# panosporf99/real-time-mobility-heatmap

Measured on AMD Instinct MI355X. Metric: events/sec H3-snapped+window-aggregated (res 8) at 1/2/4/8 GPUs; % HBM peak, higher is better.
Workload: dtype f64

## Files before the change

real-time-mobility-heatmap_amd/csrc/api_batch.h:

```cpp
#pragma once

int32_t hm_abi_version(void) { return HM_ABI_VERSION; }

int hm_create(const hm_config *cfg, hm_ctx **out) {
    g_create_err.clear();
    if (!cfg || !out) { g_create_err = "null argument"; return HM_E_INVALID; }
    if (cfg->abi_version != HM_ABI_VERSION) { g_create_err = "ABI version mismatch"; return HM_E_INVALID; }
    if (cfg->h3_res < 0 || cfg->h3_res > 15) { g_create_err = "h3_res out of range"; return HM_E_INVALID; }
    if (cfg->tile_us < 1000000 || cfg->watermark_delay_ms < 0) { g_create_err = "bad tile/watermark"; return HM_E_INVALID; }
    if (cfg->shard_count < 0 || cfg->shard_count > 64 || cfg->shard_rank < 0 ||
        (cfg->shard_count > 0 && cfg->shard_rank >= cfg->shard_count) || (cfg->shard_count == 0 && cfg->shard_rank != 0)) {
        g_create_err = "bad shard_rank/shard_count";
        return HM_E_INVALID;
    }
    int ndev = 0;
    if (hipGetDeviceCount(&ndev) != hipSuccess || ndev <= 0) {
        (void)hipGetLastError();
        g_create_err = "no HIP device available (the mobheat hot path requires an MI355X GPU)";
        return HM_E_HIP;
    }
    if (cfg->device < 0 || cfg->device >= ndev) { g_create_err = "device ordinal out of range"; return HM_E_INVALID; }
    hm_ctx *ctx = new hm_ctx();
    ctx->cfg = *cfg;
    ctx->device = cfg->device;
// ... 17 lines not shown
        if (hipEventCreate(&e) != hipSuccess) { ctx->err = "event"; return fail("create"); }
    if (hipEventCreateWithFlags(&ctx->winfo_ev, hipEventDisableTiming) != hipSuccess) { ctx->err = "event"; return fail("create"); }
    for (auto &e : ctx->h2d_ev)
        if (hipEventCreateWithFlags(&e, hipEventDisableTiming) != hipSuccess) { ctx->err = "event"; return fail("create"); }
    for (auto &e : ctx->export_ev)
        if (hipEventCreateWithFlags(&e, hipEventDisableTiming) != hipSuccess) { ctx->err = "event"; return fail("create"); }
    for (auto &e : ctx->stm_ev)
        if (hipEventCreateWithFlags(&e, hipEventDisableTiming) != hipSuccess) { ctx->err = "event"; return fail("create"); }
    if (hipFuncSetAttribute((const void *)k_merge_owned<EventRec, false>, hipFuncAttributeMaxDynamicSharedMemorySize, MO_TAG_MAX) != hipSuccess ||
        hipFuncSetAttribute((const void *)k_merge_owned<EventRec, true>, hipFuncAttributeMaxDynamicSharedMemorySize, MO_TAG_MAX) != hipSuccess ||
        hipFuncSetAttribute((const void *)k_merge_owned<EventRec, true, true>, hipFuncAttributeMaxDynamicSharedMemorySize, MO_TAG_MAX) != hipSuccess ||
        hipFuncSetAttribute((const void *)k_merge_owned<SortedRec, true, true>, hipFuncAttributeMaxDynamicSharedMemorySize, MO_TAG_MAX) != hipSuccess ||
        hipFuncSetAttribute((const void *)k_merge_owned<SortedRec, false>, hipFuncAttributeMaxDynamicSharedMemorySize, MO_TAG_MAX) != hipSuccess ||
        hipFuncSetAttribute((const void *)k_merge_owned<SortedRec, true>, hipFuncAttributeMaxDynamicSharedMemorySize, MO_TAG_MAX) != hipSuccess ||
        hipFuncSetAttribute((const void *)k_merge_owned<EventRec, false, false, true>, hipFuncAttributeMaxDynamicSharedMemorySize, MO_TAG_MAX) != hipSuccess ||
        hipFuncSetAttribute((const void *)k_merge_owned<EventRec, true, false, true>, hipFuncAttributeMaxDynamicSharedMemorySize, MO_TAG_MAX) != hipSuccess ||
        hipFuncSetAttribute((const void *)k_merge_owned<EventRec, true, true, true>, hipFuncAttributeMaxDynamicSharedMemorySize, MO_TAG_MAX) != hipSuccess) {
        ctx->err = "merge LDS attribute";
        return fail("create");
    }
    for (auto &e : ctx->ev)
        if (hipEventCreate(&e) != hipSuccess) { ctx->err = "event"; return fail("create"); }
    if (upload_tables() != hipSuccess) { ctx->err = "tables"; return fail("create"); }
    for (int variant = 0; variant < 2; variant++) {
        const void *kern = variant ? (const void *)k_ingest<true> : (const void *)k_ingest<false>;
        int per_cu = 0, cus = 0;
        if (hipOccupancyMaxActiveBlocksPerMultiprocessor(&per_cu, kern, IG_THREADS, 0) != hipSuccess ||
            hipDeviceGetAttribute(&cus, hipDeviceAttributeMultiprocessorCount, ctx->device) != hipSuccess) {
            ctx->err = "occupancy query";
            return fail("create");
        }
        hipFuncAttributes fa{};
        if (hipFuncGetAttributes(&fa, kern) == hipSuccess && fa.sharedSizeBytes > 0)
            per_cu = std::min<int>(per_cu, (int)(163840 / fa.sharedSizeBytes));
        if (variant) per_cu = std::min(per_cu, 2);
        if (const char *m = getenv("MOBHEAT_INGEST_WG_PER_CU")) {
            int w = 0, cap = 0;
            (void)hipOccupancyMaxActiveBlocksPerMultiprocessor(&cap, kern, IG_THREADS, 0);
            if (fa.sharedSizeBytes > 0) cap = std::min<int>(cap, (int)(163840 / fa.sharedSizeBytes));
            w = atoi(m);
            if (w > 0) per_cu = std::max(1, std::min(cap, w));
        }
        if (getenv("MOBHEAT_DEBUG"))
            fprintf(stderr, "mobheat: k_ingest<%d> %d blocks/CU x %d CUs (LDS %zu B, %d VGPRs)\n", variant, per_cu, cus,
                    fa.sharedSizeBytes, fa.numRegs);
        (variant ? ctx->ingest_grid_bin : ctx->ingest_grid) = std::max(1, per_cu) * std::max(1, cus);
        ctx->n_cus = std::max(1, cus);
    }
    if (const char *m = getenv("MOBHEAT_INGEST_MODE"))
        ctx->ingest_mode = !strcmp(m, "direct") ? 1 : !strcmp(m, "table") ? 2 : !strcmp(m, "binned") ? 3 : 0;
    if (const char *m = getenv("MOBHEAT_MERGE_GRID")) ctx->merge_grid = std::max(0, atoi(m));
    if (const char *m = getenv("MOBHEAT_DEDUP_STREAM")) ctx->dedup_main = !strcmp(m, "main");
    if (const char *m = getenv("MOBHEAT_DEDUP_EARLY")) ctx->early_ok = strcmp(m, "0") != 0;
    if (const char *m = getenv("MOBHEAT_OFFSETS_EARLY")) ctx->offsets_early = strcmp(m, "0") != 0;
    if (const char *m = getenv("MOBHEAT_STAGE_SELF")) ctx->self_hold_ok = strcmp(m, "copy") != 0;
    if (const char *m = getenv("MOBHEAT_DEDUP_DENSE")) ctx->dense_ok = strcmp(m, "0") != 0;
    if (const char *m = getenv("MOBHEAT_COOP_PREDICT")) ctx->coop_predict = strcmp(m, "0") != 0;
    if (const char *m = getenv("MOBHEAT_SUBBINS")) ctx->subbins_mode = !strcmp(m, "0") ? 0 : !strcmp(m, "1") ? 1 : 2;
    if (const char *m = getenv("MOBHEAT_PIPELINE")) ctx->pipe_mode = !strcmp(m, "auto") ? -1 : std::max(0, std::min(atoi(m), hm_ctx::PIPE_MAX));
    if (const char *m = getenv("MOBHEAT_TEST_SLAB_CAP")) ctx->test_slab_cap = (unsigned)std::max(0, atoi(m));
    if (hipMalloc(&ctx->d_wreg, REG_BLOCK_BYTES) != hipSuccess || !(ctx->d_wcount = ctx->d_wreg + WREG_SLOTS + 1) ||
        !(ctx->d_st = (DevStats *)(ctx->d_wreg + 2 * (WREG_SLOTS + 1))) ||
        hipHostMalloc(&ctx->h_wreg, REG_BLOCK_BYTES, hipHostMallocDefault) != hipSuccess ||
        !(ctx->h_wcount = ctx->h_wreg + WREG_SLOTS + 1) || !(ctx->h_st = (DevStats *)(ctx->h_wreg + 2 * (WREG_SLOTS + 1))) ||
        hipMalloc(&ctx->d_winfo, (WREG_SLOTS + 1) * sizeof(WInfo) + sizeof(WiCacheImg)) != hipSuccess ||
        hipHostMalloc(&ctx->h_winfo, (WREG_SLOTS + 1) * sizeof(WInfo) + sizeof(WiCacheImg), hipHostMallocDefault) != hipSuccess ||
        hipMemset(ctx->d_winfo, 0, (WREG_SLOTS + 1) * sizeof(WInfo)) != hipSuccess ||
        hipMemset(ctx->d_winfo + WREG_SLOTS + 1, 0xff, sizeof(WiCacheImg)) != hipSuccess) {
        ctx->err = "window registry alloc";
        return fail("create");
// ... 125 lines not shown
    if (ctx->stream) (void)hipStreamDestroy(ctx->stream);
    delete ctx;
}

const char *hm_last_error(const hm_ctx *ctx) { return ctx ? ctx->err.c_str() : g_create_err.c_str(); }

int hm_last_timings(const hm_ctx *ctx, double *ms, int32_t n) {
    if (!ctx || !ms) return HM_E_INVALID;
    for (int i = 0; i < n && i < 8; i++) ms[i] = ctx->timings[i];
    for (int i = 8; i < n && i < 14; i++) ms[i] = ctx->host_ms[i - 8];
    return HM_OK;
}

int64_t hm_state_version(const hm_ctx *ctx) { return ctx ? (int64_t)ctx->seq : -1; }

int hm_last_counts(const hm_ctx *ctx, int64_t *c, int32_t n) {
    if (!ctx || !c) return HM_E_INVALID;
    for (int i = 0; i < n && i < 6; i++) c[i] = ctx->last_counts[i];
    if (n > 6) c[6] = ctx->n_allocs;
    if (n > 7) c[7] = ctx->n_frees;
    if (n > 8) c[8] = ctx->last_binned;
    if (n > 9) c[9] = ctx->staged ? ctx->stage_self_recs : 0;
    if (n > 10) c[10] = ctx->staged ? 0 : ctx->last_pipe_chunks;
    return HM_OK;
}


int hm_process_batch(hm_ctx *ctx, int64_t epoch_id, const hm_batch_in *in, int32_t out_memory, hm_batch_out *out) {
    if (!ctx || !in || !out || in->n < 0) return ctx ? set_err(ctx, HM_E_INVALID, "bad argument") : HM_E_INVALID;
    if (in->n > MAX_BATCH_ROWS) return set_err(ctx, HM_E_INVALID, "batch of %lld events exceeds %lld", (long long)in->n, (long long)MAX_BATCH_ROWS);
    if (in->n > 0 && (!in->lat || !in->lon || !in->ts_us || !in->vkey))
        return set_err(ctx, HM_E_INVALID, "lat, lon, ts_us and vkey are required");
    if (ctx->shard_count > 1)
        return set_err(ctx, HM_E_STATE, "a context of shard %d of %d runs the stage API (its state is that shard's keys)",
                       ctx->shard_rank, ctx->shard_count);
    HIPCHK(ctx, hipSetDevice(ctx->device));
    host_batch_begin(ctx);
    const BatchClock clock_(ctx);
    memset(out, 0, sizeof(*out));
    ctx->gmap_ready = false;
    ctx->epoch = epoch_id;
    ctx->last_n_latest = -1;
    ctx->staged = false;
    ctx->stage = 0;
    int rc;
    int64_t late_wm = ctx->cfg.late_uses_prev_watermark ? ctx->wm_prev : ctx->wm_cur;
    Inputs I;
    I.n = in->n;
    if ((rc = stage_inputs(ctx, in, &I.lat, &I.lon, &I.ts, &I.sp, &I.sv, &I.vk, &I.rv))) return rc;
    const bool sub = ctx->subbins_mode == 1 || (ctx->subbins_mode == 2 && ctx->merge_coop);
    const bool early = ctx->early_ok && !ctx->dedup_main;
    const int K = pipe_chunks_for(ctx, I);
    bool piped = false;
    ctx->last_pipe_chunks = 0;
    if (K > 1) {
        bool to_table = false;
        if ((rc = process_pipelined(ctx, I, late_wm, sub, K, early, to_table))) return rc;
        piped = !to_table;
    } else if ((rc = phase_local(ctx, I, late_wm, true, sub, early, ctx->offsets_early))) {
        return rc;
    }
    DevStats s1 = *ctx->h_st;
    const int64_t n_agg = (int64_t)s1.n_valid - (int64_t)s1.n_late;
    const bool table = !piped && choose_table(ctx, n_agg, s1.sample_max_run);
    ctx->last_table = table;
    ctx->dedup_side = s1.dedup_retry == 0 && !ctx->dedup_main;
    if (ctx->dedup_early && !ctx->dedup_side)
        HIPCHK(ctx, hipStreamWaitEvent(ctx->stream, ctx->side_ev[2], 0));
    if (ctx->dedup_side && !ctx->dedup_early) {
        HIPCHK(ctx, hipEventRecord(ctx->side_ev[0], ctx->stream));
        HIPCHK(ctx, hipStreamWaitEvent(ctx->side_stream, ctx->side_ev[0], 0));
        if ((rc = launch_side_dedup(ctx, &I))) return rc;
    }
    if (table) {
        int64_t n_parts = 0;
        if ((rc = phase_table(ctx, I, n_agg, &n_parts))) return rc;
        HIPCHK(ctx, hipEventRecord(ctx->ev[2], ctx->stream));
        if ((rc = merge_partials(ctx, (const TilePartial *)ctx->partials.p, n_parts))) return rc;
    } else if (!piped) {
        HIPCHK(ctx, hipEventRecord(ctx->ev[2], ctx->stream));
        if ((rc = merge_events(ctx, I, n_agg))) return rc;
    }
    if (!ctx->dedup_side) {
        if ((rc = phase_dedup(ctx, &I, nullptr, I.n, true))) return rc;
    } else {
// ... 38 lines not shown
```

real-time-mobility-heatmap_amd/csrc/host_batch.h:

```cpp
#pragma once

constexpr int64_t BIN_MIN_ROWS = int64_t(1) << 22;
static bool prev_says_table(const hm_ctx *ctx) {
    return ctx->prev_keys > 0 && ctx->prev_keys <= (int64_t)AG_BINS * (AG_SLOTS / 2) && ctx->prev_agg_rows >= 8 * ctx->prev_keys;
}
static bool choose_binned(const hm_ctx *ctx, int64_t n) {
    if (ctx->ingest_mode) return ctx->ingest_mode == 3;
    return n >= BIN_MIN_ROWS && !prev_says_table(ctx);
}
static unsigned slab_cap_for(int64_t n, double skew, int64_t nbins) {
    const int64_t m = (n + nbins - 1) / nbins;
    const int64_t c = std::min<int64_t>(std::max<int64_t>(m + m / 4 + 256, (int64_t)(skew * 1.1 * (double)m) + 256), n + 256);
    return (unsigned)std::min<int64_t>((c + 1) & ~int64_t(1), (int64_t)UINT32_MAX / 2);
}

static int launch_side_dedup(hm_ctx *ctx, const Inputs *I);
static int bin_offsets(hm_ctx *ctx);
static int prepare_local(hm_ctx *ctx, int64_t n, int64_t late_wm_ms, bool bin, bool sub) {
    int rc;
    if (ctx->dedup_early) HIPCHK(ctx, hipStreamWaitEvent(ctx->stream, ctx->side_ev[2], 0));
    ctx->dedup_early = false;
    if ((rc = ensure(ctx, ctx->flags, n)) || (rc = ensure(ctx, ctx->win, n)) || (rc = ensure(ctx, ctx->rows, n * 8)) ||
        (rc = ensure(ctx, ctx->keys, n * 8)) || (rc = ensure(ctx, ctx->slow, n * sizeof(unsigned int))))
        return rc;
// ... 12 lines not shown
        }
    }
    ctx->keys_partial = bin;
    ctx->keys_late_us = late_wm_ms * 1000;
    ctx->sub_bits = bin && sub ? SUB_BITS : 0;
    const int nbins = RP_BINS << ctx->sub_bits;
    ctx->slab_cap = bin ? slab_cap_for(n, ctx->bin_skew, nbins) : 0;
    if (bin && ctx->test_slab_cap) ctx->slab_cap = std::min(ctx->slab_cap, ctx->test_slab_cap);
    ctx->binned = false;
    ctx->bin_offsets_ready = false;
    if ((rc = ensure(ctx, ctx->bin_cur, ((RP_BINS << SUB_BITS) + 1) * 4))) return rc;
    if (bin && (rc = ensure(ctx, ctx->parts_sorted, ((size_t)nbins * ctx->slab_cap + 64) * sizeof(EventRec)))) return rc;
    {
        const int nw = 2 * (WREG_SLOTS + 1);
        hipLaunchKernelGGL(k_batch_reset, dim3((std::max(nw, nbins + 1) + 255) / 256), dim3(256), 0, ctx->stream,
                           (unsigned long long *)ctx->d_st, ctx->d_scratch + SLOW_WORD, ctx->d_scratch + GIVEUP_WORD, ctx->d_wreg,
                           nw, (unsigned *)ctx->bin_cur.p, nbins + 1);
        HIPCHK(ctx, hipGetLastError());
    }
    return HM_OK;
}

static void launch_ingest(hm_ctx *ctx, const Inputs &I, int64_t a, int64_t b, bool bin, int64_t late_wm_ms) {
    const int blocks = (int)std::min<int64_t>((b - a + IG_THREADS - 1) / IG_THREADS, bin ? ctx->ingest_grid_bin : ctx->ingest_grid);
    auto kern = bin ? k_ingest<true> : k_ingest<false>;
    hipLaunchKernelGGL(kern, dim3(std::max(blocks, 1)), dim3(IG_THREADS), 0, ctx->stream, I.lat, I.lon, I.ts, I.rv, I.vk, a, b,
                       ctx->cfg.h3_res, make_floor_div(ctx->cfg.tile_us), late_wm_ms * 1000, (uint8_t *)ctx->flags.p,
                       (uint64_t *)ctx->keys.p, ctx->dfused.tab, ctx->dfused.cap - 1, (unsigned int *)ctx->dfused.used.p,
                       ctx->d_scratch + ctx->dfused.used_word, (unsigned int *)ctx->slow.p, ctx->d_scratch + SLOW_WORD,
                       ctx->d_scratch + GIVEUP_WORD, ctx->d_wreg, ctx->d_wcount, ctx->d_st, I.sp, I.sv,
                       (unsigned *)ctx->bin_cur.p, bin ? (EventRec *)ctx->parts_sorted.p : nullptr, ctx->slab_cap,
                       (unsigned long long *)ctx->dense.p, ctx->dense_cap, ctx->sub_bits, hs_stride(I.n) - 1);
}

static int phase_local(hm_ctx *ctx, const Inputs &I, int64_t late_wm_ms, bool allow_bin = false, bool sub = false,
                       bool early_dedup = false, bool offsets = false) {
    int64_t n = I.n;
    int rc;
    const bool bin = allow_bin && n > 0 && choose_binned(ctx, n);
    if ((rc = prepare_local(ctx, n, late_wm_ms, bin, sub))) return rc;
    const int nbins = RP_BINS << ctx->sub_bits;
    HIPCHK(ctx, hipEventRecord(ctx->ev[0], ctx->stream));
    if (n > 0) {
        const int nch = ctx->n_h2d ? (int)std::min<int64_t>(hm_ctx::H2D_CHUNKS, std::max<int64_t>(1, n >> 22)) : 1;
        if (ctx->n_h2d) {
            HIPCHK(ctx, hipEventRecord(ctx->h2d_ev[0], ctx->stream));
            HIPCHK(ctx, hipStreamWaitEvent(ctx->copy_stream, ctx->h2d_ev[0], 0));
        }
        for (int c = 0; c < nch; c++) {
            const int64_t a = n * c / nch, b = n * (c + 1) / nch;
            if (ctx->n_h2d) {
                for (int q = 0; q < ctx->n_h2d; q++) {
                    const hm_ctx::H2D &h = ctx->h2d[q];
                    HIPCHK(ctx, hipMemcpyAsync((uint8_t *)h.dst + a * h.el, (const uint8_t *)h.src + a * h.el, (b - a) * h.el,
                                               hipMemcpyHostToDevice, ctx->copy_stream));
// ... 31 lines not shown
        unsigned long long tot = 0, mx = 0;
        for (int b = 0; b < nbins; b++) { tot += ctx->h_bincur[b]; mx = std::max<unsigned long long>(mx, ctx->h_bincur[b]); }
        if (tot) ctx->bin_skew = std::max(1.0, (double)mx * nbins / (double)tot);
    }
    if (ctx->h_st->win_overflow)
        return set_err(ctx, HM_E_OVERFLOW, "more than %d distinct windows in one micro-batch (%llu rows)", WREG_SLOTS,
                       ctx->h_st->win_overflow);
    ctx->binned = bin && ctx->h_st->bin_overflow == 0;
    if (ctx->h_st->vkey_max1) ctx->vkey_bound = (int64_t)ctx->h_st->vkey_max1;
    return HM_OK;
}

static int keys_complete(hm_ctx *ctx, const Inputs &I) {
    if (!ctx->keys_partial) return HM_OK;
    ctx->keys_partial = false;
    if (I.n == 0) return HM_OK;
    const int blocks = (int)std::min<int64_t>((I.n + IG_THREADS - 1) / IG_THREADS, ctx->ingest_grid);
    hipLaunchKernelGGL((k_ingest<false, true>), dim3(blocks), dim3(IG_THREADS), 0, ctx->stream, I.lat, I.lon, I.ts, I.rv, I.vk,
                       (int64_t)0, I.n, ctx->cfg.h3_res, make_floor_div(ctx->cfg.tile_us), ctx->keys_late_us,
                       (uint8_t *)ctx->flags.p, (uint64_t *)ctx->keys.p, ctx->dfused.tab, ctx->dfused.cap - 1,
                       (unsigned int *)ctx->dfused.used.p, ctx->d_scratch + ctx->dfused.used_word, (unsigned int *)ctx->slow.p,
                       ctx->d_scratch + SLOW_WORD, ctx->d_scratch + GIVEUP_WORD, ctx->d_wreg, ctx->d_wcount, ctx->d_st, I.sp,
                       I.sv, (unsigned *)ctx->bin_cur.p, (EventRec *)nullptr, 0u, (unsigned long long *)ctx->dense.p, 0ull, 0u,
                       (int64_t)0);
    HIPCHK(ctx, hipGetLastError());
    return HM_OK;
}

static bool choose_table(const hm_ctx *ctx, int64_t n_agg, unsigned long long sample_max_run) {
    if (ctx->ingest_mode) return ctx->ingest_mode == 2;
    if (n_agg < (int64_t(1) << 16)) return false;
    if (sample_max_run >= (unsigned long long)(HS_SAMPLE / 256)) return true;
    return prev_says_table(ctx);
}

static int phase_table(hm_ctx *ctx, const Inputs &I, int64_t n_agg, int64_t *n_parts) {
    int rc;
    const int64_t n = I.n;
    if ((rc = keys_complete(ctx, I))) return rc;
    if ((rc = ensure(ctx, ctx->partials, std::max<int64_t>(n_agg, 1) * sizeof(TilePartial)))) return rc;
    const int nsub = AG_BINS * AG_SUB;
    if (ctx->agg_cap == 0)
        ctx->agg_cap = (unsigned)std::min<int64_t>(std::max<int64_t>(4096, n_agg / (2 * nsub)), int64_t(1) << 30);
    if ((rc = ensure(ctx, ctx->agg_bucket, (size_t)nsub * ctx->agg_cap * sizeof(AggRec))) ||
        (rc = ensure(ctx, ctx->agg_cursor, (size_t)nsub * 8)))
        return rc;
    HIPCHK(ctx, hipMemsetAsync(ctx->agg_cursor.p, 0, (size_t)nsub * 8, ctx->stream));
// ... 278 lines not shown
```

real-time-mobility-heatmap_amd/csrc/host_ctx.h:

```cpp
#pragma once

struct DevBuf {
    void *p = nullptr;
    size_t bytes = 0;
};

struct Inputs {
    const double *lat, *lon, *sp;
    const int64_t *ts;
    const uint8_t *sv, *rv;
    const uint64_t *vk;
    int64_t n;
};

struct hm_ctx {
    hm_config cfg;
    int device = 0;
    hipStream_t stream = nullptr;
    std::string err;
    hipEvent_t ev[11] = {};
    static constexpr int H2D_CHUNKS = 16;
    hipStream_t copy_stream = nullptr;
    hipStream_t side_stream = nullptr;
    hipEvent_t side_ev[4] = {};
// ... 33 lines not shown
    unsigned long long export_dump_seq = 0;
    static constexpr int STM_PIECES = 64;
    hipEvent_t stm_ev[STM_PIECES] = {};
    int stm_pieces = 0;
    int64_t stm_piece = 0, stm_total = 0;
    static constexpr int EXPORT_SLICES = 64;
    hipEvent_t export_ev[EXPORT_SLICES] = {};
    DevBuf parts_regrow_sorted;
    DevBuf stage_meta, stage_C, stage_P, stage_SO, stage_SP, stage_T, cands_recv, stage_tmp;
    DevBuf gapbuf;
    unsigned long long seq = 0;
    struct DedupTable {
        DedupSlot *tab = nullptr;
        unsigned long long cap = 0;
        DevBuf used;
        bool dirty = false;
        int used_word = 0;
    } dfused, dfull;
    DedupTable *dlast = nullptr;
    int64_t dedup_seen = 0;
    int64_t n_partials_merged = 0;
    int ingest_grid = 0;
    int ingest_grid_bin = 0;
    int64_t last_binned = 0;
    int n_cus = 0;
    int ingest_mode = 0;
    int merge_grid = 0;
    int64_t prev_agg_rows = 0, prev_keys = 0;
    bool merge_coop = false;
    bool coop_predict = true;
    bool last_table = false;
    int64_t last_counts[6] = {0, 0, 0, 0, 0, 0};
    int64_t n_allocs = 0, n_frees = 0;
    int64_t table_evicted = 0;
    struct Dict {
        DevBuf tab, slot_of, occ, slots, code_of_slot, clen, coff, cbytes, btot, boff;
        int64_t last_codes = 0;
        int64_t n_codes = 0;
        void *h_off = nullptr, *h_bytes = nullptr;
        size_t h_off_cap = 0, h_bytes_cap = 0;
    };
    DevBuf jd_bytes, jd_offs, jd_scratch, jd_lat, jd_lon, jd_ts, jd_speed, jd_sv, jd_rv, jd_vkey, jd_poff, jd_plen, jd_voff,
        jd_vlen, jd_un, jd_unrows, jd_patch;
    std::vector<int64_t> jd_unsup;
    int64_t jd_n = -1, jd_np = 0, jd_nv = 0;
    Dict jd_prov, jd_veh;
// ... 808 lines not shown
```

real-time-mobility-heatmap_amd/csrc/host_pipe.h:

```cpp
#pragma once

constexpr int PIPE_CHUNKS = 4;
constexpr int64_t PIPE_MIN_ROWS = int64_t(1) << 24;

static int pipe_chunks_for(const hm_ctx *ctx, const Inputs &I) {
    if (ctx->pipe_mode == 0 || I.n <= 0) return 0;
    if (!choose_binned(ctx, I.n)) return 0;
    if (ctx->pipe_mode > 0) return ctx->pipe_mode >= 2 && I.n >= ctx->pipe_mode ? ctx->pipe_mode : 0;
    return I.n >= PIPE_MIN_ROWS ? PIPE_CHUNKS : 0;
}

static bool g_pipe_debug = getenv("MOBHEAT_PIPE_DEBUG") && getenv("MOBHEAT_PIPE_DEBUG")[0] == '1';
#define PIPE_STEP(ctx, what, k)                                                                                   \
    do {                                                                                                          \
        if (g_pipe_debug) {                                                                                       \
            const hipError_t e_ = hipDeviceSynchronize();                                                         \
            const hipError_t l_ = hipGetLastError();                                                              \
            fprintf(stderr, "[mobheat pipe] %s chunk %d: %s\n", what, (int)(k), hipGetErrorString(e_ ? e_ : l_)); \
            if (e_ || l_) return set_err(ctx, HM_E_HIP, "pipelined batch: %s of chunk %d: %s", what, (int)(k),  \
                                         hipGetErrorString(e_ ? e_ : l_));                                        \
        }                                                                                                         \
    } while (0)

static hipError_t ev_sync(hm_ctx *ctx, hipEvent_t e, int site) {
// ... 37 lines not shown
    return HM_OK;
}

static void pipe_batch_stats(hm_ctx *ctx, int nbins) {
    unsigned long long tot = 0, mx = 0;
    for (int b = 0; b < nbins; b++) { tot += ctx->h_bincur[b]; mx = std::max<unsigned long long>(mx, ctx->h_bincur[b]); }
    if (tot) ctx->bin_skew = std::max(1.0, (double)mx * nbins / (double)tot);
    if (ctx->h_st->vkey_max1) ctx->vkey_bound = (int64_t)ctx->h_st->vkey_max1;
}

static int pipe_overflow_rest(hm_ctx *ctx, const Inputs &I, int K, int k) {
    int rc;
    const int64_t n = I.n, a = n * k / K;
    unsigned long long *plO = (unsigned long long *)ctx->pl_O.p;
    unsigned *plN = (unsigned *)ctx->pl_cnt.p;
    HIPCHK(ctx, hipStreamSynchronize(ctx->merge_stream));
    const int blocks = (int)std::min<int64_t>((n - a + IG_THREADS - 1) / IG_THREADS, ctx->ingest_grid);
    hipLaunchKernelGGL((k_ingest<false, true>), dim3(std::max(blocks, 1)), dim3(IG_THREADS), 0, ctx->stream, I.lat, I.lon, I.ts,
                       I.rv, I.vk, a, n, ctx->cfg.h3_res, make_floor_div(ctx->cfg.tile_us), ctx->keys_late_us,
                       (uint8_t *)ctx->flags.p, (uint64_t *)ctx->keys.p, ctx->dfused.tab, ctx->dfused.cap - 1,
                       (unsigned int *)ctx->dfused.used.p, ctx->d_scratch + ctx->dfused.used_word, (unsigned int *)ctx->slow.p,
                       ctx->d_scratch + SLOW_WORD, ctx->d_scratch + GIVEUP_WORD, ctx->d_wreg, ctx->d_wcount, ctx->d_st, I.sp,
                       I.sv, (unsigned *)ctx->bin_cur.p, (EventRec *)nullptr, 0u, (unsigned long long *)ctx->dense.p, 0ull, 0u,
                       (int64_t)0);
    HIPCHK(ctx, hipGetLastError());
    PIPE_STEP(ctx, "overflow: keys", k);
    ctx->keys_partial = false;
    if (k == 0) {
        int r;
        if ((r = merge_begin(ctx, n, true))) return r;
        HIPCHK(ctx, hipEventRecord(ctx->ev[3], ctx->stream));
    } else if ((rc = gens_sync_counts(ctx))) {
        return rc;
    }
    std::vector<WinCount> census;
    census_of_registry(ctx, census);
    ctx->batch_windows.clear();
    if ((rc = gens_prepare(ctx, census, true)) || (rc = winfo_upload(ctx, true))) return rc;
    Inputs Ik = I;
    Ik.lat += a; Ik.lon += a; Ik.ts += a; Ik.vk += a;
    if (Ik.sp) Ik.sp += a;
    if (Ik.sv) Ik.sv += a;
    if (Ik.rv) Ik.rv += a;
    Ik.n = n - a;
    int64_t ntiles = 1;
    PIPE_STEP(ctx, "overflow: tables", k);
    if ((rc = ev_partition(ctx, (const uint64_t *)ctx->keys.p + a, n - a, &Ik, ntiles))) return rc;
// ... 203 lines not shown
```

real-time-mobility-heatmap_amd/csrc/k_ingest.h:

```cpp
#pragma once

#define HM_SNAP_ATTR __attribute__((amdgpu_waves_per_eu(6)))
__global__ __launch_bounds__(256) void k_cells(const double *__restrict__ lat, const double *__restrict__ lon, int64_t n,
                                               int res, uint64_t *__restrict__ out, unsigned int *__restrict__ slow,
                                               unsigned long long *n_slow) {
    const int64_t stride = (int64_t)gridDim.x * blockDim.x;
    for (int64_t base = (int64_t)blockIdx.x * blockDim.x; base < n; base += stride) {
        const int64_t i = base + threadIdx.x;
        bool exc = false;
        if (i < n) {
            uint64_t c;
            exc = !latLngToCellFast(lat[i], lon[i], res, c_tab, c);
            out[i] = c;
        }
        const unsigned long long pos = wave_append(exc, n_slow);
        if (exc) slow[pos] = (unsigned int)i;
    }
}
__global__ __launch_bounds__(256) void k_cells_exact(const double *__restrict__ lat, const double *__restrict__ lon,
                                                     int res, uint64_t *__restrict__ out, const unsigned int *__restrict__ slow,
                                                     const unsigned long long *n_slow) {
    const int64_t m = (int64_t)*n_slow;
    for (int64_t q = (int64_t)blockIdx.x * blockDim.x + threadIdx.x; q < m; q += (int64_t)gridDim.x * blockDim.x) {
        const unsigned i = slow[q];
        out[i] = latLngToCellDeg(lat[i], lon[i], res, c_tab);
    }
}

constexpr unsigned long long DEDUP_FUSED_PROBES = 32;
constexpr int IG_THREADS = 256;

__device__ __forceinline__ void wave_count_slots(bool pred, int slot, unsigned *cnt) {
    unsigned long long pend = __ballot(pred);
    while (pend) {
        const int leader = __ffsll((long long)pend) - 1;
        const int s = __shfl(slot, leader, 64);
        const unsigned long long m = __ballot(pred && slot == s);
        if (lane_id() == leader) atomicAdd(&cnt[s], (unsigned)__popcll(m));
        pend &= ~m;
    }
}

constexpr int HS_SAMPLE = 4096, HS_THREADS = 1024, HS_SLOTS = 2 * HS_SAMPLE;
__host__ __device__ inline int64_t hs_stride(int64_t n) {
    int64_t s = 1;
    while (s * 2 <= n / HS_SAMPLE) s *= 2;
    return s;
}
template <bool kBin, bool kKeys = false>
__global__ __launch_bounds__(IG_THREADS) HM_SNAP_ATTR void k_ingest(
    const double *__restrict__ lat, const double *__restrict__ lon, const int64_t *__restrict__ ts,
    const uint8_t *__restrict__ row_valid, const uint64_t *__restrict__ vkey, int64_t i_begin, int64_t n, int res_arg, FloorDiv wdiv,
    int64_t late_end_us, uint8_t *__restrict__ flags_out, uint64_t *__restrict__ keys_out, DedupSlot *dtab,
    unsigned long long dmask, unsigned int *dused, unsigned long long *n_dused, unsigned int *__restrict__ slow,
    unsigned long long *n_slow, unsigned long long *dgiveup, unsigned long long *wreg, unsigned long long *wcount,
    DevStats *st, const double *__restrict__ speed, const uint8_t *__restrict__ speed_valid, unsigned *__restrict__ bin_cur,
    EventRec *__restrict__ slabs, unsigned slab_cap, unsigned long long *__restrict__ dense, unsigned long long dense_cap,
    unsigned sub_bits, int64_t smask) {
    static_assert(!(kBin && kKeys), "k_ingest: kKeys runs unbinned");
    const int res = res_arg;
    __shared__ WinCacheL WC;
    __shared__ double Fc[20][3], Fu[20][2][3];
    __shared__ unsigned dskip;
    __shared__ long long tmax_l[IG_THREADS];
    __shared__ long long vmax_l[IG_THREADS];
    for (int k = threadIdx.x; k < 60; k += IG_THREADS) (&Fc[0][0])[k] = (&c_tab.faceCenterPoint[0][0])[k];
    for (int k = threadIdx.x; k < 120; k += IG_THREADS) (&Fu[0][0][0])[k] = (&c_tab.fastU[res & 1][0][0][0])[k];
    __shared__ H3BaseTables BT;
    for (int k = threadIdx.x; k < 20 * 27; k += IG_THREADS) BT.fijkPacked[k] = c_tab.fijkPacked[k];
    for (int k = threadIdx.x; k < 122; k += IG_THREADS) BT.bcdPacked[k] = c_tab.bcdPacked[k];
    for (int k = threadIdx.x; k < AP7_QUAD; k += IG_THREADS) BT.ap7Quad[k] = c_tab.ap7Quad[k];
    for (int k = threadIdx.x; k < AP7_PAIR; k += IG_THREADS) BT.ap7Pair[k] = c_tab.ap7Pair[k];
    wc_init(WC);
    if (threadIdx.x == 0) dskip = 0;
    __syncthreads();
    const int64_t tile_us = wdiv.d;
    unsigned nvalid = 0, nlate = 0, bad = 0, wover = 0, binover = 0;
    tmax_l[threadIdx.x] = INT64_MIN;
    vmax_l[threadIdx.x] = 0;
    bool dretry = false;
    int round = 0;
    const int64_t gstride = (int64_t)gridDim.x * IG_THREADS;
    double nla = 0.0, nlo = 0.0;
    int64_t nt = 0;
    unsigned long long nv = EMPTY_VKEY;
    uint8_t nrv = 1;
    {
        const int64_t i0 = i_begin + (int64_t)blockIdx.x * IG_THREADS + threadIdx.x;
        if (i0 < n) {
            nla = __builtin_nontemporal_load(&lat[i0]);
            nlo = __builtin_nontemporal_load(&lon[i0]);
            nv = __builtin_nontemporal_load(&vkey[i0]);
            if (row_valid) nrv = __builtin_nontemporal_load(&row_valid[i0]);
        }
    }
    for (int64_t base = i_begin + (int64_t)blockIdx.x * IG_THREADS; base < n; base += gstride, round++) {
        const int64_t i = base + threadIdx.x;
        const bool in = i < n;
        const double la = nla, lo = nlo;
        const int64_t t = in ? __builtin_nontemporal_load(&ts[i]) : 0;
        (void)nt;
        uint64_t spb = 0;
        uint8_t svb = 0;
        if constexpr (kBin) {
            typedef __attribute__((address_space(1))) const uint64_t gcu64;
            typedef __attribute__((address_space(1))) const uint8_t gcu8;
            const int64_t j = in ? i : n - 1;
            spb = __builtin_nontemporal_load((gcu64 *)(speed ? (const uint64_t *)&speed[j] : (const uint64_t *)&g_zero_double));
            svb = __builtin_nontemporal_load((gcu8 *)(speed_valid ? &speed_valid[j] : speed ? &g_one_byte : &g_zero_byte));
        }
        const unsigned long long v = nv;
        const bool rv = nrv != 0;
        {
            const int64_t j = i + gstride < n ? i + gstride : n - 1;
            nla = __builtin_nontemporal_load(&lat[j]);
            nlo = __builtin_nontemporal_load(&lon[j]);
            nv = __builtin_nontemporal_load(&vkey[j]);
            nrv = __builtin_nontemporal_load(
                (__attribute__((address_space(1))) const uint8_t *)(row_valid ? &row_valid[j] : &g_one_byte));
// ... 42 lines not shown
        if (dd && dv) {
            const long long cur = (long long)(dn ^ DENSE_SIGN);
            cand = t >= cur;
            if (t > cur) atomicMax(&dense[v], (unsigned long long)t ^ DENSE_SIGN);
        } else if (dd) {
            long long cur = d0.maxts;
            if (d0.vkey == v) dh = (long long)dh0;
            else dh = find_or_claim_vkey_ts(dtab, dmask, v, claimed, DEDUP_FUSED_PROBES, cur);
            if (dh < 0) {
                if (!dretry) atomicExch(dgiveup, 1ull);
                dretry = true;
            } else {
                cand = t >= cur || claimed;
                if (t > cur) atomicMax(&dtab[dh].maxts, (long long)t);
            }
        }
        const bool agg = (fl & F_AGG) != 0;
        const uint64_t key = agg ? ekey_make(exc ? 0 : cell, (unsigned)widx) : 0;
        if (in) {
            if constexpr (!kKeys) flags_out[i] = fl | (cand ? F_CAND : 0);
            if (kKeys ? !exc : !kBin || exc || (i & smask) == 0) keys_out[i] = key;
        }
        if constexpr (kBin) {
            if (agg && !exc) {
                uint64_t inner = wslot >= 0 ? __hip_atomic_load(&WC.inner[wslot], __ATOMIC_RELAXED, __HIP_MEMORY_SCOPE_WORKGROUP) : 0;
                if (inner == 0) {
                    inner = window_inner(ws);
                    if (wslot >= 0) __hip_atomic_store(&WC.inner[wslot], inner, __ATOMIC_RELAXED, __HIP_MEMORY_SCOPE_WORKGROUP);
                }
                const uint64_t h = mix64(cell ^ inner);
                const unsigned b = (region_field(h) << sub_bits) | (sub_field(h) & ((1u << sub_bits) - 1));
                const unsigned p = atomicAdd(&bin_cur[b], 1u);
                if (p < slab_cap) {
                    const uint64_t sp = svb == 0 ? SPEED_NULL_BITS
                                                 : __builtin_bit_cast(double, spb) != __builtin_bit_cast(double, spb) ? CANON_NAN_BITS : spb;
                    const uint64_t lab = __builtin_bit_cast(uint64_t, la), lob = __builtin_bit_cast(uint64_t, lo);
                    uint4 *d = (uint4 *)&slabs[(size_t)b * slab_cap + p];
                    st_g16(d, make_uint4((unsigned)key, (unsigned)(key >> 32), (unsigned)sp, (unsigned)(sp >> 32)));
                    st_g16(d + 1, make_uint4((unsigned)lab, (unsigned)(lab >> 32), (unsigned)lob, (unsigned)(lob >> 32)));
                } else {
                    binover++;
                }
            }
        }
        if constexpr (!kKeys) {
            const unsigned long long pos = wave_append(claimed, n_dused);
            if (claimed) dused[pos] = (unsigned int)dh;
            wave_count_slots(agg && wslot >= 0, wslot, WC.cnt);
            if (agg && wslot < 0) atomicAdd(&wcount[widx], 1ull);
        }
        if (threadIdx.x == 0 && (round & 15) == 15 && !dskip)
            __hip_atomic_store(&dskip, __hip_atomic_load(dgiveup, __ATOMIC_RELAXED, __HIP_MEMORY_SCOPE_AGENT) != 0 ? 1u : 0u,
                               __ATOMIC_RELAXED, __HIP_MEMORY_SCOPE_WORKGROUP);
    }
    if constexpr (kKeys) return;
    __syncthreads();
    for (int q = threadIdx.x; q < WC_SLOTS; q += IG_THREADS)
        if (WC.cnt[q]) atomicAdd(&wcount[(WC.e[q] & 0xfff) - 1], (unsigned long long)WC.cnt[q]);
    const unsigned long long wvalid = wave_sum((unsigned long long)nvalid), wlate = wave_sum((unsigned long long)nlate);
    const unsigned long long wbad = wave_sum((unsigned long long)bad), wwover = wave_sum((unsigned long long)wover);
    const unsigned long long wbinover = kBin ? wave_sum((unsigned long long)binover) : 0ull;
    const long long tmax = wave_max(tmax_l[threadIdx.x]);
    const long long vmax = wave_max(vmax_l[threadIdx.x]);
    const unsigned long long rt = __ballot(dretry);
    if (lane_id() == 0) {
        if (wvalid) atomicAdd(&st->n_valid, wvalid);
        if (wlate) atomicAdd(&st->n_late, wlate);
        if (tmax != INT64_MIN) atomicMax(&st->max_ts_ms, (long long)(tmax / 1000));
        if (vmax > 0) atomicMax(&st->vkey_max1, (unsigned long long)vmax);
        if (wbad) atomicAdd(&st->bad_vkey, wbad);
        if (wwover) atomicAdd(&st->win_overflow, wwover);
        if (rt) atomicAdd(&st->dedup_retry, 1ull);
        if (wbinover) atomicAdd(&st->bin_overflow, wbinover);
    }
}


__global__ __launch_bounds__(256) void k_ingest_exact(const double *__restrict__ lat, const double *__restrict__ lon, int res,
                                                      const unsigned int *__restrict__ slow, const unsigned long long *n_slow,
                                                      uint64_t *__restrict__ keys, const double *__restrict__ speed,
// ... 77 lines not shown
```

real-time-mobility-heatmap_amd/csrc/kernels.h:

```cpp
#pragma once
#include <hip/hip_runtime.h>
#include <stdint.h>

#include "h3_device.h"

namespace hm {

constexpr uint64_t EMPTY_CELL = 0;
constexpr int64_t EMPTY_WIN = INT64_MIN;
constexpr uint64_t EMPTY_VKEY = ~UINT64_C(0);
constexpr int WAVE = 64;

enum : uint8_t { F_VALID = 1, F_AGG = 2, F_LATE = 4, F_CAND = 8 };

struct alignas(64) TileSlot {
    uint64_t cell;
    unsigned long long wenc;
    unsigned long long count;
    unsigned long long nspeed;
    double sspeed;
    double slat;
    double slon;
    unsigned long long touched;
};
// ... 112 lines not shown
    long long maxts;
};

struct DevStats {
    unsigned long long n_valid;
    unsigned long long n_late;
    long long max_ts_ms;
    long long min_wstart;
    unsigned long long n_partials;
    unsigned long long n_touched;
    unsigned long long n_state_new;
    unsigned long long n_dedup_used;
    unsigned long long n_cands;
    unsigned long long overflow;
    unsigned long long bad_vkey;
    unsigned long long dedup_retry;
    unsigned long long n_gaps;
    unsigned long long win_overflow;
    unsigned long long agg_spill;
    unsigned long long n_evicted;
    unsigned long long sample_max_run;
    unsigned long long bin_overflow;
    unsigned long long vkey_max1;
};

constexpr unsigned long long DENSE_SIGN = 0x8000000000000000ull;

HM_HD uint64_t mix64(uint64_t x) {
    x ^= x >> 33;
    x *= UINT64_C(0xff51afd7ed558ccd);
    x ^= x >> 33;
    x *= UINT64_C(0xc4ceb9fe1a85ec53);
    x ^= x >> 33;
    return x;
}
HM_HD uint64_t window_inner(int64_t w) { return mix64((uint64_t)w + UINT64_C(0x9e3779b97f4a7c15)); }
HM_HD uint64_t tile_hash(uint64_t cell, int64_t w) { return mix64(cell ^ window_inner(w)); }
struct FloorDiv {
    uint64_t m;
    int s1, s2;
    int64_t d;
};
HM_HD uint64_t umulhi64(uint64_t a, uint64_t b) {
#if defined(__HIP_DEVICE_COMPILE__)
    return __umul64hi(a, b);
#else
// ... 40 lines not shown
```

Baseline: 10.81 billion.

## Add dedicated writer waves draining LDS rings for binned ingest scatter

In binned ingest mode, producer waves now push computed records into per-wave LDS ring buffers instead of doing the global bin atomic and slab store themselves. Two extra writer waves per workgroup drain the rings in batches and perform the atomics and 32-byte slab writes. The goal is to overlap the scattered global writes with H3 snapping compute. The cost is extra LDS, a larger workgroup, lower waves-per-EU (5 instead of 6), and polling/sleep overhead, with a direct-write fallback when a ring is full.

```diff
diff --git a/real-time-mobility-heatmap_amd/csrc/api_batch.h b/real-time-mobility-heatmap_amd/csrc/api_batch.h
--- a/real-time-mobility-heatmap_amd/csrc/api_batch.h
+++ b/real-time-mobility-heatmap_amd/csrc/api_batch.h
@@ -63,10 +63,20 @@
     for (auto &e : ctx->ev)
         if (hipEventCreate(&e) != hipSuccess) { ctx->err = "event"; return fail("create"); }
     if (upload_tables() != hipSuccess) { ctx->err = "tables"; return fail("create"); }
+    ctx->ingest_writers = true;
+    ctx->ring_polls = IGW_RING_POLLS;
+    if (const char *m = getenv("MOBHEAT_INGEST_WRITERS")) ctx->ingest_writers = strcmp(m, "0") != 0;
+    if (const char *m = getenv("MOBHEAT_TEST_RING_POLLS")) ctx->ring_polls = (unsigned)std::max(0, atoi(m));
+    ctx->ring_cap = IGW_RING;
+    if (const char *m = getenv("MOBHEAT_TEST_RING_CAP")) ctx->ring_cap = (unsigned)std::max(0, std::min(atoi(m), IGW_RING));
     for (int variant = 0; variant < 2; variant++) {
-        const void *kern = variant ? (const void *)k_ingest<true> : (const void *)k_ingest<false>;
+        const bool wr = variant && ctx->ingest_writers;
+        const void *kern = wr        ? (const void *)k_ingest<true, false, IGW_WRITERS, IGW_ROUNDS, IGW_PROD>
+                           : variant ? (const void *)k_ingest<true>
+                                     : (const void *)k_ingest<false>;
+        const int threads = wr ? (IGW_PROD + IGW_WRITERS) * 64 : IG_THREADS;
         int per_cu = 0, cus = 0;
-        if (hipOccupancyMaxActiveBlocksPerMultiprocessor(&per_cu, kern, IG_THREADS, 0) != hipSuccess ||
+        if (hipOccupancyMaxActiveBlocksPerMultiprocessor(&per_cu, kern, threads, 0) != hipSuccess ||
             hipDeviceGetAttribute(&cus, hipDeviceAttributeMultiprocessorCount, ctx->device) != hipSuccess) {
             ctx->err = "occupancy query";
             return fail("create");
@@ -77,16 +87,20 @@
         if (variant) per_cu = std::min(per_cu, 2);
         if (const char *m = getenv("MOBHEAT_INGEST_WG_PER_CU")) {
             int w = 0, cap = 0;
-            (void)hipOccupancyMaxActiveBlocksPerMultiprocessor(&cap, kern, IG_THREADS, 0);
+            (void)hipOccupancyMaxActiveBlocksPerMultiprocessor(&cap, kern, threads, 0);
             if (fa.sharedSizeBytes > 0) cap = std::min<int>(cap, (int)(163840 / fa.sharedSizeBytes));
             w = atoi(m);
             if (w > 0) per_cu = std::max(1, std::min(cap, w));
         }
         if (getenv("MOBHEAT_DEBUG"))
-            fprintf(stderr, "mobheat: k_ingest<%d> %d blocks/CU x %d CUs (LDS %zu B, %d VGPRs)\n", variant, per_cu, cus,
-                    fa.sharedSizeBytes, fa.numRegs);
+            fprintf(stderr, "mobheat: k_ingest<%d>%s %d blocks/CU of %d threads x %d CUs (LDS %zu B, %d VGPRs)\n", variant,
+                    wr ? " (writer waves)" : "", per_cu, threads, cus, fa.sharedSizeBytes, fa.numRegs);
         (variant ? ctx->ingest_grid_bin : ctx->ingest_grid) = std::max(1, per_cu) * std::max(1, cus);
         ctx->n_cus = std::max(1, cus);
+    }
+    if (const char *m = getenv("MOBHEAT_TEST_INGEST_GRID")) {
+        const int g = atoi(m);
+        if (g > 0) { ctx->ingest_grid = std::min(ctx->ingest_grid, g); ctx->ingest_grid_bin = std::min(ctx->ingest_grid_bin, g); }
     }
     if (const char *m = getenv("MOBHEAT_INGEST_MODE"))
         ctx->ingest_mode = !strcmp(m, "direct") ? 1 : !strcmp(m, "table") ? 2 : !strcmp(m, "binned") ? 3 : 0;
@@ -258,6 +272,7 @@
     if (n > 8) c[8] = ctx->last_binned;
     if (n > 9) c[9] = ctx->staged ? ctx->stage_self_recs : 0;
     if (n > 10) c[10] = ctx->staged ? 0 : ctx->last_pipe_chunks;
+    if (n > 11) c[11] = ctx->last_ring_direct;
     return HM_OK;
 }
 
@@ -297,6 +312,7 @@
         return rc;
     }
     DevStats s1 = *ctx->h_st;
+    ctx->last_ring_direct = (int64_t)s1.ring_direct;
     const int64_t n_agg = (int64_t)s1.n_valid - (int64_t)s1.n_late;
     const bool table = !piped && choose_table(ctx, n_agg, s1.sample_max_run);
     ctx->last_table = table;
diff --git a/real-time-mobility-heatmap_amd/csrc/host_batch.h b/real-time-mobility-heatmap_amd/csrc/host_batch.h
--- a/real-time-mobility-heatmap_amd/csrc/host_batch.h
+++ b/real-time-mobility-heatmap_amd/csrc/host_batch.h
@@ -58,15 +58,18 @@
 }
 
 static void launch_ingest(hm_ctx *ctx, const Inputs &I, int64_t a, int64_t b, bool bin, int64_t late_wm_ms) {
-    const int blocks = (int)std::min<int64_t>((b - a + IG_THREADS - 1) / IG_THREADS, bin ? ctx->ingest_grid_bin : ctx->ingest_grid);
-    auto kern = bin ? k_ingest<true> : k_ingest<false>;
-    hipLaunchKernelGGL(kern, dim3(std::max(blocks, 1)), dim3(IG_THREADS), 0, ctx->stream, I.lat, I.lon, I.ts, I.rv, I.vk, a, b,
+    const bool wr = bin && ctx->ingest_writers;
+    const int rows = wr ? IGW_PROD * 64 : IG_THREADS, threads = wr ? (IGW_PROD + IGW_WRITERS) * 64 : IG_THREADS;
+    const int blocks = (int)std::min<int64_t>((b - a + rows - 1) / rows, bin ? ctx->ingest_grid_bin : ctx->ingest_grid);
+    auto kern = wr ? k_ingest<true, false, IGW_WRITERS, IGW_ROUNDS, IGW_PROD> : bin ? k_ingest<true> : k_ingest<false>;
+    hipLaunchKernelGGL(kern, dim3(std::max(blocks, 1)), dim3(threads), 0, ctx->stream, I.lat, I.lon, I.ts, I.rv, I.vk, a, b,
                        ctx->cfg.h3_res, make_floor_div(ctx->cfg.tile_us), late_wm_ms * 1000, (uint8_t *)ctx->flags.p,
                        (uint64_t *)ctx->keys.p, ctx->dfused.tab, ctx->dfused.cap - 1, (unsigned int *)ctx->dfused.used.p,
                        ctx->d_scratch + ctx->dfused.used_word, (unsigned int *)ctx->slow.p, ctx->d_scratch + SLOW_WORD,
                        ctx->d_scratch + GIVEUP_WORD, ctx->d_wreg, ctx->d_wcount, ctx->d_st, I.sp, I.sv,
                        (unsigned *)ctx->bin_cur.p, bin ? (EventRec *)ctx->parts_sorted.p : nullptr, ctx->slab_cap,
-                       (unsigned long long *)ctx->dense.p, ctx->dense_cap, ctx->sub_bits, hs_stride(I.n) - 1);
+                       (unsigned long long *)ctx->dense.p, ctx->dense_cap, ctx->sub_bits, hs_stride(I.n) - 1, ctx->ring_polls,
+                       ctx->ring_cap);
 }
 
 static int phase_local(hm_ctx *ctx, const Inputs &I, int64_t late_wm_ms, bool allow_bin = false, bool sub = false,
@@ -144,7 +147,7 @@
                        (unsigned int *)ctx->dfused.used.p, ctx->d_scratch + ctx->dfused.used_word, (unsigned int *)ctx->slow.p,
                        ctx->d_scratch + SLOW_WORD, ctx->d_scratch + GIVEUP_WORD, ctx->d_wreg, ctx->d_wcount, ctx->d_st, I.sp,
                        I.sv, (unsigned *)ctx->bin_cur.p, (EventRec *)nullptr, 0u, (unsigned long long *)ctx->dense.p, 0ull, 0u,
-                       (int64_t)0);
+                       (int64_t)0, 0u, 0u);
     HIPCHK(ctx, hipGetLastError());
     return HM_OK;
 }
diff --git a/real-time-mobility-heatmap_amd/csrc/host_ctx.h b/real-time-mobility-heatmap_amd/csrc/host_ctx.h
--- a/real-time-mobility-heatmap_amd/csrc/host_ctx.h
+++ b/real-time-mobility-heatmap_amd/csrc/host_ctx.h
@@ -79,6 +79,10 @@
     int64_t n_partials_merged = 0;
     int ingest_grid = 0;
     int ingest_grid_bin = 0;
+    bool ingest_writers = false;
+    unsigned ring_polls = 0;
+    unsigned ring_cap = 0;
+    int64_t last_ring_direct = 0;
     int64_t last_binned = 0;
     int n_cus = 0;
     int ingest_mode = 0;
diff --git a/real-time-mobility-heatmap_amd/csrc/host_pipe.h b/real-time-mobility-heatmap_amd/csrc/host_pipe.h
--- a/real-time-mobility-heatmap_amd/csrc/host_pipe.h
+++ b/real-time-mobility-heatmap_amd/csrc/host_pipe.h
@@ -83,7 +83,7 @@
                        (unsigned int *)ctx->dfused.used.p, ctx->d_scratch + ctx->dfused.used_word, (unsigned int *)ctx->slow.p,
                        ctx->d_scratch + SLOW_WORD, ctx->d_scratch + GIVEUP_WORD, ctx->d_wreg, ctx->d_wcount, ctx->d_st, I.sp,
                        I.sv, (unsigned *)ctx->bin_cur.p, (EventRec *)nullptr, 0u, (unsigned long long *)ctx->dense.p, 0ull, 0u,
-                       (int64_t)0);
+                       (int64_t)0, 0u, 0u);
     HIPCHK(ctx, hipGetLastError());
     PIPE_STEP(ctx, "overflow: keys", k);
     ctx->keys_partial = false;
diff --git a/real-time-mobility-heatmap_amd/csrc/k_ingest.h b/real-time-mobility-heatmap_amd/csrc/k_ingest.h
--- a/real-time-mobility-heatmap_amd/csrc/k_ingest.h
+++ b/real-time-mobility-heatmap_amd/csrc/k_ingest.h
@@ -1,6 +1,7 @@
 #pragma once
 
-#define HM_SNAP_ATTR __attribute__((amdgpu_waves_per_eu(6)))
+constexpr int ig_waves_per_simd(int writers) { return writers ? 5 : 6; }
+#define HM_SNAP_ATTR __attribute__((amdgpu_waves_per_eu(ig_waves_per_simd(0))))
 __global__ __launch_bounds__(256) void k_cells(const double *__restrict__ lat, const double *__restrict__ lon, int64_t n,
                                                int res, uint64_t *__restrict__ out, unsigned int *__restrict__ slow,
                                                unsigned long long *n_slow) {
@@ -47,8 +48,90 @@
     while (s * 2 <= n / HS_SAMPLE) s *= 2;
     return s;
 }
-template <bool kBin, bool kKeys = false>
-__global__ __launch_bounds__(IG_THREADS) HM_SNAP_ATTR void k_ingest(
+constexpr int IGW_RING = 128;
+constexpr int IGW_PROD = 8;
+constexpr int IGW_WRITERS = 2, IGW_ROUNDS = 4;
+constexpr unsigned IGW_RING_POLLS = 256;
+struct IngestRing {
+    unsigned long long key[IGW_RING], sp[IGW_RING], la[IGW_RING], lo[IGW_RING];
+    unsigned bin[IGW_RING];
+    unsigned tail, head, done;
+};
+template <int kProd>
+struct IngestRings { IngestRing r[kProd]; };
+template <>
+struct IngestRings<0> {};
+__device__ __forceinline__ unsigned ring_word(const unsigned *w) {
+    return __builtin_amdgcn_readfirstlane(__hip_atomic_load(w, __ATOMIC_RELAXED, __HIP_MEMORY_SCOPE_WORKGROUP));
+}
+__device__ __forceinline__ void ring_acquire() { __builtin_amdgcn_fence(__ATOMIC_ACQUIRE, "workgroup", "local"); }
+__device__ __forceinline__ void ring_publish(unsigned *w, unsigned v) {
+    __builtin_amdgcn_fence(__ATOMIC_RELEASE, "workgroup", "local");
+    if (lane_id() == 0) __hip_atomic_store(w, v, __ATOMIC_RELAXED, __HIP_MEMORY_SCOPE_WORKGROUP);
+}
+template <int kProd, int kWriters, int kRounds>
+__device__ __forceinline__ unsigned ingest_writer(IngestRings<kProd> &RG, int wj, unsigned *__restrict__ bin_cur,
+                                                  EventRec *__restrict__ slabs, unsigned slab_cap) {
+    constexpr int NQ = (kProd + kWriters - 1) / kWriters;
+    const unsigned ln = (unsigned)lane_id();
+    unsigned over = 0;
+    int cur = wj;
+    for (;;) {
+        unsigned cnt[kRounds], b[kRounds], p[kRounds];
+        uint64_t key[kRounds], sp[kRounds], la[kRounds], lo[kRounds];
+#pragma unroll
+        for (int r = 0; r < kRounds; r++) {
+            cnt[r] = 0;
+            b[r] = p[r] = 0;
+            key[r] = sp[r] = la[r] = lo[r] = 0;
+            for (int tries = 0; tries < NQ && cnt[r] == 0; tries++) {
+                IngestRing &Q = RG.r[cur];
+                cur = cur + kWriters < kProd ? cur + kWriters : wj;
+                const unsigned d = ring_word(&Q.done);
+                ring_acquire();
+                const unsigned t = ring_word(&Q.tail), h = ring_word(&Q.head);
+                ring_acquire();
+                const unsigned avail = t - h, take = avail >= 64 ? 64u : d ? avail : 0u;
+                if (take == 0) continue;
+                if (ln < take) {
+                    const unsigned s = (h + ln) & (IGW_RING - 1);
+                    b[r] = Q.bin[s];
+                    key[r] = Q.key[s];
+                    sp[r] = Q.sp[s];
+                    la[r] = Q.la[s];
+                    lo[r] = Q.lo[s];
+                }
+                ring_publish(&Q.head, h + take);
+                cnt[r] = take;
+            }
+            if (ln < cnt[r]) p[r] = atomicAdd(&bin_cur[b[r]], 1u);
+        }
+#pragma unroll
+        for (int r = 0; r < kRounds; r++) {
+            if (ln >= cnt[r]) continue;
+            if (p[r] < slab_cap) {
+                uint4 *d = (uint4 *)&slabs[(size_t)b[r] * slab_cap + p[r]];
+                st_g16(d, make_uint4((unsigned)key[r], (unsigned)(key[r] >> 32), (unsigned)sp[r], (unsigned)(sp[r] >> 32)));
+                st_g16(d + 1, make_uint4((unsigned)la[r], (unsigned)(la[r] >> 32), (unsigned)lo[r], (unsigned)(lo[r] >> 32)));
+            } else {
+                over++;
+            }
+        }
+        if (cnt[0]) continue;
+        bool fin = true;
+        for (int q = wj; q < kProd; q += kWriters) {
+            const unsigned d = ring_word(&RG.r[q].done);
+            ring_acquire();
+            fin = fin && d && ring_word(&RG.r[q].tail) == ring_word(&RG.r[q].head);
+        }
+        if (fin) break;
+        __builtin_amdgcn_s_sleep(8);
+    }
+    return over;
+}
+
+template <bool kBin, bool kKeys = false, int kWriters = 0, int kRounds = 1, int kProd = IG_THREADS / 64>
+__global__ __launch_bounds__((kProd + kWriters) * 64) __attribute__((amdgpu_waves_per_eu(ig_waves_per_simd(kWriters)))) void k_ingest(
     const double *__restrict__ lat, const double *__restrict__ lon, const int64_t *__restrict__ ts,
     const uint8_t *__restrict__ row_valid, const uint64_t *__restrict__ vkey, int64_t i_begin, int64_t n, int res_arg, FloorDiv wdiv,
     int64_t late_end_us, uint8_t *__restrict__ flags_out, uint64_t *__restrict__ keys_out, DedupSlot *dtab,
@@ -56,21 +139,29 @@
     unsigned long long *n_slow, unsigned long long *dgiveup, unsigned long long *wreg, unsigned long long *wcount,
     DevStats *st, const double *__restrict__ speed, const uint8_t *__restrict__ speed_valid, unsigned *__restrict__ bin_cur,
     EventRec *__restrict__ slabs, unsigned slab_cap, unsigned long long *__restrict__ dense, unsigned long long dense_cap,
-    unsigned sub_bits, int64_t smask) {
+    unsigned sub_bits, int64_t smask, unsigned ring_polls, unsigned ring_cap) {
     static_assert(!(kBin && kKeys), "k_ingest: kKeys runs unbinned");
+    static_assert(kWriters == 0 ? kProd * 64 == IG_THREADS : kBin, "k_ingest: writer waves belong to the binned kernel");
+    constexpr int kRows = kProd * 64, kThreads = (kProd + kWriters) * 64;
+    const int wave = __builtin_amdgcn_readfirstlane((int)(threadIdx.x >> 6));
+    const bool writer = kWriters > 0 && wave >= kProd;
+    __shared__ IngestRings<kWriters ? kProd : 0> RG;
+    if constexpr (kWriters > 0)
+        if (threadIdx.x < kProd) RG.r[threadIdx.x].tail = RG.r[threadIdx.x].head = RG.r[threadIdx.x].done = 0;
+    unsigned ring_tail = 0;
     const int res = res_arg;
     __shared__ WinCacheL WC;
     __shared__ double Fc[20][3], Fu[20][2][3];
     __shared__ unsigned dskip;
-    __shared__ long long tmax_l[IG_THREADS];
-    __shared__ long long vmax_l[IG_THREADS];
-    for (int k = threadIdx.x; k < 60; k += IG_THREADS) (&Fc[0][0])[k] = (&c_tab.faceCenterPoint[0][0])[k];
-    for (int k = threadIdx.x; k < 120; k += IG_THREADS) (&Fu[0][0][0])[k] = (&c_tab.fastU[res & 1][0][0][0])[k];
+    __shared__ long long tmax_l[kThreads];
+    __shared__ long long vmax_l[kThreads];
+    for (int k = threadIdx.x; k < 60; k += kThreads) (&Fc[0][0])[k] = (&c_tab.faceCenterPoint[0][0])[k];
+    for (int k = threadIdx.x; k < 120; k += kThreads) (&Fu[0][0][0])[k] = (&c_tab.fastU[res & 1][0][0][0])[k];
     __shared__ H3BaseTables BT;
-    for (int k = threadIdx.x; k < 20 * 27; k += IG_THREADS) BT.fijkPacked[k] = c_tab.fijkPacked[k];
-    for (int k = threadIdx.x; k < 122; k += IG_THREADS) BT.bcdPacked[k] = c_tab.bcdPacked[k];
-    for (int k = threadIdx.x; k < AP7_QUAD; k += IG_THREADS) BT.ap7Quad[k] = c_tab.ap7Quad[k];
-    for (int k = threadIdx.x; k < AP7_PAIR; k += IG_THREADS) BT.ap7Pair[k] = c_tab.ap7Pair[k];
+    for (int k = threadIdx.x; k < 20 * 27; k += kThreads) BT.fijkPacked[k] = c_tab.fijkPacked[k];
+    for (int k = threadIdx.x; k < 122; k += kThreads) BT.bcdPacked[k] = c_tab.bcdPacked[k];
+    for (int k = threadIdx.x; k < AP7_QUAD; k += kThreads) BT.ap7Quad[k] = c_tab.ap7Quad[k];
+    for (int k = threadIdx.x; k < AP7_PAIR; k += kThreads) BT.ap7Pair[k] = c_tab.ap7Pair[k];
     wc_init(WC);
     if (threadIdx.x == 0) dskip = 0;
     __syncthreads();
@@ -80,21 +171,21 @@
     vmax_l[threadIdx.x] = 0;
     bool dretry = false;
     int round = 0;
-    const int64_t gstride = (int64_t)gridDim.x * IG_THREADS;
+    const int64_t gstride = (int64_t)gridDim.x * kRows;
     double nla = 0.0, nlo = 0.0;
     int64_t nt = 0;
     unsigned long long nv = EMPTY_VKEY;
     uint8_t nrv = 1;
     {
-        const int64_t i0 = i_begin + (int64_t)blockIdx.x * IG_THREADS + threadIdx.x;
-        if (i0 < n) {
+        const int64_t i0 = i_begin + (int64_t)blockIdx.x * kRows + threadIdx.x;
+        if (i0 < n && !writer) {
             nla = __builtin_nontemporal_load(&lat[i0]);
             nlo = __builtin_nontemporal_load(&lon[i0]);
             nv = __builtin_nontemporal_load(&vkey[i0]);
             if (row_valid) nrv = __builtin_nontemporal_load(&row_valid[i0]);
         }
     }
-    for (int64_t base = i_begin + (int64_t)blockIdx.x * IG_THREADS; base < n; base += gstride, round++) {
+    for (int64_t base = writer ? n : i_begin + (int64_t)blockIdx.x * kRows; base < n; base += gstride, round++) {
         const int64_t i = base + threadIdx.x;
         const bool in = i < n;
         const double la = nla, lo = nlo;
@@ -183,19 +274,52 @@
             if (kKeys ? !exc : !kBin || exc || (i & smask) == 0) keys_out[i] = key;
         }
         if constexpr (kBin) {
-            if (agg && !exc) {
+            const bool rec = agg && !exc;
+            unsigned b = 0;
+            if (rec) {
                 uint64_t inner = wslot >= 0 ? __hip_atomic_load(&WC.inner[wslot], __ATOMIC_RELAXED, __HIP_MEMORY_SCOPE_WORKGROUP) : 0;
                 if (inner == 0) {
                     inner = window_inner(ws);
                     if (wslot >= 0) __hip_atomic_store(&WC.inner[wslot], inner, __ATOMIC_RELAXED, __HIP_MEMORY_SCOPE_WORKGROUP);
                 }
                 const uint64_t h = mix64(cell ^ inner);
-                const unsigned b = (region_field(h) << sub_bits) | (sub_field(h) & ((1u << sub_bits) - 1));
+                b = (region_field(h) << sub_bits) | (sub_field(h) & ((1u << sub_bits) - 1));
+            }
+            const uint64_t sp = svb == 0 ? SPEED_NULL_BITS
+                                         : __builtin_bit_cast(double, spb) != __builtin_bit_cast(double, spb) ? CANON_NAN_BITS : spb;
+            const uint64_t lab = __builtin_bit_cast(uint64_t, la), lob = __builtin_bit_cast(uint64_t, lo);
+            bool direct = rec;
+            if constexpr (kWriters > 0) {
+                const unsigned long long m = __ballot(rec);
+                if (m) {
+                    IngestRing &Q = RG.r[wave];
+                    const unsigned cnt = (unsigned)__popcll(m);
+                    bool room = ring_tail + cnt - ring_word(&Q.head) <= ring_cap;
+                    for (unsigned q = 0; !room && q < ring_polls; q++) {
+                        __builtin_amdgcn_s_sleep(4);
+                        room = ring_tail + cnt - ring_word(&Q.head) <= ring_cap;
+                    }
+                    if (room) {
+                        ring_acquire();
+                        if (rec) {
+                            const unsigned s = (ring_tail + (unsigned)__popcll(m & ((1ull << lane_id()) - 1))) & (IGW_RING - 1);
+                            Q.bin[s] = b;
+                            Q.key[s] = key;
+                            Q.sp[s] = sp;
+                            Q.la[s] = lab;
+                            Q.lo[s] = lob;
+                        }
+                        ring_tail += cnt;
+                        ring_publish(&Q.tail, ring_tail);
+                        direct = false;
+                    } else if (lane_id() == 0) {
+                        atomicAdd(&st->ring_direct, (unsigned long long)cnt);
+                    }
+                }
+            }
+            if (direct) {
                 const unsigned p = atomicAdd(&bin_cur[b], 1u);
                 if (p < slab_cap) {
-                    const uint64_t sp = svb == 0 ? SPEED_NULL_BITS
-                                                 : __builtin_bit_cast(double, spb) != __builtin_bit_cast(double, spb) ? CANON_NAN_BITS : spb;
-                    const uint64_t lab = __builtin_bit_cast(uint64_t, la), lob = __builtin_bit_cast(uint64_t, lo);
                     uint4 *d = (uint4 *)&slabs[(size_t)b * slab_cap + p];
                     st_g16(d, make_uint4((unsigned)key, (unsigned)(key >> 32), (unsigned)sp, (unsigned)(sp >> 32)));
                     st_g16(d + 1, make_uint4((unsigned)lab, (unsigned)(lab >> 32), (unsigned)lob, (unsigned)(lob >> 32)));
@@ -215,8 +339,12 @@
                                __ATOMIC_RELAXED, __HIP_MEMORY_SCOPE_WORKGROUP);
     }
     if constexpr (kKeys) return;
+    if constexpr (kWriters > 0) {
+        if (writer) binover = ingest_writer<kProd, kWriters, kRounds>(RG, wave - kProd, bin_cur, slabs, slab_cap);
+        else ring_publish(&RG.r[wave].done, 1u);
+    }
     __syncthreads();
-    for (int q = threadIdx.x; q < WC_SLOTS; q += IG_THREADS)
+    for (int q = threadIdx.x; q < WC_SLOTS; q += kThreads)
         if (WC.cnt[q]) atomicAdd(&wcount[(WC.e[q] & 0xfff) - 1], (unsigned long long)WC.cnt[q]);
     const unsigned long long wvalid = wave_sum((unsigned long long)nvalid), wlate = wave_sum((unsigned long long)nlate);
     const unsigned long long wbad = wave_sum((unsigned long long)bad), wwover = wave_sum((unsigned long long)wover);
diff --git a/real-time-mobility-heatmap_amd/csrc/kernels.h b/real-time-mobility-heatmap_amd/csrc/kernels.h
--- a/real-time-mobility-heatmap_amd/csrc/kernels.h
+++ b/real-time-mobility-heatmap_amd/csrc/kernels.h
@@ -158,6 +158,7 @@
     unsigned long long sample_max_run;
     unsigned long long bin_overflow;
     unsigned long long vkey_max1;
+    unsigned long long ring_direct;
 };
 
 constexpr unsigned long long DENSE_SIGN = 0x8000000000000000ull;
```

Result: faster. 11.24 billion, median of 6 (+4.0%).
